# akshilpatel/tile-match-gym

Hardware: AMD Instinct MI355X
Metric: env-steps/sec (whole node), 65536×10×10 boards, at 1/2/4/8 MI355X (higher is better)
Workload: dtype int8; 1 GPU; c2: 65536 x 10x10 boards per GPU, 4 colours, no specials, num_moves=30, autoreset, 3 episode-phase blocks offset by 10 steps, the timed window opening on a block's reset step (phases + 4); boards_per_gpu=65536, rows=10, cols=10, colours=4, env_groups_per_gpu=3, phase_blocks=3, policy=uniform, api=raw, graph=False, parallelism=dp1 (independent env shards, no collective)

## Files before the change

tile-match-gym_amd/csrc/tmg_board.hip:

```cpp
#include <hip/hip_runtime.h>
#include <stdint.h>

#include "pcg64.h"

namespace tmg {

#define WSYNC() __syncthreads()

#ifndef TMG_LEAN128_WAVES
#define TMG_LEAN128_WAVES 8
#endif
constexpr int kLean128Waves = TMG_LEAN128_WAVES;
constexpr int kLean128GenericWaves = 7;
constexpr int kGen128Waves = 5;
#ifndef TMG_RESET512_WAVES
#define TMG_RESET512_WAVES 8
#endif
#ifndef TMG_RESET128_WAVES
#define TMG_RESET128_WAVES 8
#endif
constexpr int kReset512Waves = TMG_RESET512_WAVES;
constexpr int kReset128Waves = TMG_RESET128_WAVES;
#ifndef TMG_PEEK_LEAN_WAVES
#define TMG_PEEK_LEAN_WAVES 5
// ... 53 lines not shown
    CV_SPILL,
    CV_SPILL_RUN,
    CV_SHUFFLE,
    CV_REJECT,
    CV_FAST,
    CV_SHUFFLE_GEN,
    CV_REJECT_GEN,
    CV_RP_PASSES,
    CV_RP_PERP,
    CV_RP_VLONG,
    CV_RP_WIDE,
    CV_RP_REJECT,
    CV_LANE_STEP,
    CV_LANE_SHUFFLE,
    CV_LANE_REDRAW,
    CV_LANE_REJECT,
    CV_LANE_REJECT_REDRAW,
    CV_RP_CARRY,
    CV_RP_REBATCH,
    CV_PEEK_MOVE,
    CV_PEEK_SPILL,
    CV_PEEK_SPILL_RUN,
    CV_ROLL_PLY,
    CV_ROLL_HORIZON,
    CV_ROLL_SPILL,
    CV_ROLL_SPILL_RUN,
    CV_BP_PAIR_ACC,
    CV_BP_PAIR_REJ,
    CV_RP_VSHIFT,
    CV_RP_VMORE,
    CV_RP_SCAN2,
    CV_BP_ROUND_CARRY,
    CV_RP_NOLDS,
    CV_COUNT = 48
};
#if TMG_COVER
#define COVER(site)                                                                                     \
    do {                                                                                                \
        if (lane == 0 && P.cover) atomicAdd(P.cover + (site), 1ULL);                                   \
    } while (0)
#define COVER_L0(site)                                                                                  \
    do {                                                                                                \
        if (P.cover) atomicAdd(P.cover + (site), 1ULL);                                                \
    } while (0)
#else
#define COVER(site) ((void)0)
#define COVER_L0(site) ((void)0)
#endif

struct Params {
    int R, C, N, A, W, k, smask, num_moves;
    uint32_t thr;
    uint32_t cmag, cm1mag;
    const uint64_t *jump;
    uint64_t sb_nl[2];
    uint64_t sb_nf[2];
    uint64_t sb_h[2];
    uint64_t sb_z;
    uint64_t sb_in[2], sb_u[2], sb_v[2];
    const uint64_t *sb_rows;
    uint32_t *status;
    void *oh;
    int oh_dtype, oh_ch, oh_nsel;
    uint32_t oh_sel;
    SpillQ *spill;
    void *spill_ws;
    unsigned long long *cover;
// ... 2148 lines not shown
    return elim;
}

struct JumpRow { uint64_t a0, a1, g0, g1; };
__device__ __forceinline__ JumpRow jump_row_load(const Params &P, int l, bool rowp) {
    const uint64_t *t = P.jump + (rowp ? bp_out(l) : l) * 4;
    return JumpRow{t[0], t[1], t[2], t[3]};
}
__device__ __forceinline__ LaneJump jump_row_finish(const JumpRow &r, const Rng &g) {
    LaneJump J;
    J.Aj = U128{r.a0, r.a1};
    J.Gj = U128{r.g0, r.g1};
    J.incG = mul128(U128{g.ilo, g.ihi}, J.Gj);
    return J;
}
__device__ __forceinline__ LaneJump load_jump(const Params &P, int lane, const Rng &g, bool rowp = false) {
    return jump_row_finish(jump_row_load(P, lane, rowp), g);
}
__device__ __forceinline__ LaneJump load_jump_bp(const Params &P, int lane, const Rng &g) {
    return load_jump(P, lane, g, true);
}

__device__ __forceinline__ Rng load_rng(const uint64_t *p) {
    Rng g;
    g.slo = bcast64(p[0]); g.shi = bcast64(p[1]); g.ilo = bcast64(p[2]); g.ihi = bcast64(p[3]); g.h = bcast64(p[4]);
    return g;
}
__device__ __forceinline__ void store_rng(uint64_t *p, const Rng &g, int lane) {
    if (lane == 0) { p[0] = g.slo; p[1] = g.shi; p[2] = g.ilo; p[3] = g.ihi; p[4] = g.h; }
}

#include "tmg_rp.hip"

template <int MAXN, bool GEN, int SBNB, bool CODD, int TIER = TIER_MAIN, class WS = Ws<MAXN, GEN>,
          class L = WsSerial<MAXN>, bool FIXED = false>
__device__ __forceinline__ uint32_t step_env(
    const Params &P, WS &w, int lane, int64_t e, int8_t *__restrict__ board, uint64_t *__restrict__ rng, int32_t *__restrict__ timer,
    const int32_t *__restrict__ actions, int32_t *__restrict__ reward, int32_t *__restrict__ n_new,
    int32_t *__restrict__ n_act, uint8_t *__restrict__ flags_out, uint64_t *__restrict__ eff, int trust_eff,
    int autoreset, L *lists) {
    const int N = P.N, W = P.W;
    constexpr bool INLINE_GEN = !GEN && MAXN == 128;
    const bool same = autoreset == 1 || autoreset == 2;
    const bool regen_inline = autoreset == 1 || autoreset == 3;
    int a = __builtin_amdgcn_readfirstlane(actions[e]);
    const int t0 = __builtin_amdgcn_readfirstlane(timer[e]);
    const uint64_t effrow = lane < W ? eff[e * W + lane] : 0ULL;
    TMG_KEEP_V(effrow);
    if (P.sample) {
        a = __builtin_amdgcn_readfirstlane(sample_action(P, effrow, e, lane));
        if (lane == 0) const_cast<int32_t *>(actions)[e] = a;
    }
#ifndef TMG_QEXIT
#define TMG_QEXIT 1
#endif
    if (TMG_QEXIT && trust_eff && t0 < P.num_moves - 1 && (unsigned)a < (unsigned)P.A) {
        if (!((rdlane64(effrow, a >> 6) >> (a & 63)) & 1ULL)) {
            if (lane == 0) {
                uint64_t ve = (uint64_t)e;
                TMG_OPAQUE_V(ve);
                timer[ve] = t0 + 1;
                reward[ve] = 0; n_new[ve] = 0; n_act[ve] = 0;
                flags_out[ve] = (uint8_t)0;
                if (P.vo_term) reinterpret_cast<uint32_t *>(P.vo_term)[ve] = 0u;
                if (P.vo_left) P.vo_left[ve] = (int64_t)(P.num_moves - 1 - t0);
            }
            return 0;
        }
    }
    bool pend = false;
    if (t0 >= P.num_moves || a < 0 || a >= P.A) {
        pend = autoreset >= 3 && t0 >= P.num_moves;
    }
    if (!pend && (t0 >= P.num_moves || a < 0 || a >= P.A)) {
        if (lane == 0) {
            reward[e] = 0; n_new[e] = 0; n_act[e] = 0; flags_out[e] = FL_ERR;
            store_vo(P, e, FL_ERR, t0);
        }
        if ((P.oh || P.vo_obs) && !trust_eff) {
            load_board(P, w, lane, board + e * 2 * N);
            WSYNC();
            if (P.oh) store_onehot(P, w, lane, e);
            if (P.vo_obs) store_obs(P, w, lane, e);
        }
        return ST_CALLER;
    }
    int8_t *gb = board + e * 2 * N;
    uint64_t *ge = eff + e * W;
    const int t1 = t0 + 1;
    const bool done = !pend && t1 == P.num_moves;
    const bool regen = pend || (done && same);
    int flags = done ? FL_DONE : 0;
    bool effective = false;
    if (trust_eff && !pend) {
        effective = (rdlane64(effrow, a >> 6) >> (a & 63)) & 1ULL;
    }
    if (trust_eff && !effective && !(regen && regen_inline)) {
        const bool defer = regen;
        if (done && !same) {
            for (int i = lane; i < W; i += 64) ge[i] = 0ULL;
            if (P.vo_mask) store_mask(P, w, lane, e, true);
        }
        if (done && same && P.vo_final) {
            const int nbw = ((2 * N) & 3) == 0 ? (2 * N) >> 2 : 0;
            const uint32_t *src = reinterpret_cast<const uint32_t *>(gb);
            uint32_t *dst = reinterpret_cast<uint32_t *>(P.vo_final + e * 2 * N);
            for (int i = lane; i < nbw; i += 64) dst[i] = src[i];
            for (int i = 4 * nbw + lane; i < 2 * N; i += 64) P.vo_final[e * 2 * N + i] = gb[i];
        }
        if (lane == 0) {
            const int tn = defer ? 0 : t1;
            timer[e] = tn; reward[e] = 0; n_new[e] = 0; n_act[e] = 0;
            flags_out[e] = (uint8_t)(flags | (defer ? FL_RESET : 0));
            store_vo(P, e, flags, tn);
        }
        return 0;
    }
    int r1, c1, r2, c2;
    action_coords(P.R, P.C, a, r1, c1, r2, c2);
    const int p1 = r1 * P.C + c1, p2 = r2 * P.C + c2;

    const int nbw = (2 * N) >> 2;
    const bool bwhole = ((2 * N) & 3) == 0 && nbw <= 64;
    const uint32_t bw = bwhole ? reinterpret_cast<const uint32_t *>(gb)[lane < nbw ? lane : 0] : 0u;
    const uint64_t *rp = rng + e * 5;
    const uint64_t q0 = rp[0], q1 = rp[1], q2 = rp[2], q3 = rp[3], q4 = rp[4];
    bool rowp = false;
    if constexpr (SBNB > 0 && !GEN) rowp = rp_shape(P);
    const JumpRow jrow = jump_row_load(P, lane, rowp);
    if (bwhole) {
        if (lane < nbw) reinterpret_cast<uint32_t *>(w.brd)[lane] = bw;
    } else {
        load_board(P, w, lane, gb);
    }
    if constexpr (GEN) {
        for (int p = lane; p < N; p += 64) w.mark[p] = 0;
    }
    if constexpr (TIER == TIER_SPILL) COVER(CV_SPILL_RUN);
    WSYNC();
    if constexpr (!GEN) {
        bool ok = true;
        for (int p = lane; p < N; p += 64) ok &= w.brd[N + p] == 1;
        if (__ballot(!ok) != 0ULL) {
            if (lane == 0) {
                reward[e] = 0; n_new[e] = 0; n_act[e] = 0; flags_out[e] = FL_ERR;
                store_vo(P, e, FL_ERR, t0);
            }
            return ST_INTERNAL;
        }
    }
    if (!trust_eff && !pend) {
        bool ex = lane == 0 ? eff_exact(P, w.brd, a) : false;
        effective = __ballot(ex) != 0ULL;
    }
    Rng g;
    g.slo = bcast64(q0); g.shi = bcast64(q1); g.ilo = bcast64(q2); g.ihi = bcast64(q3); g.h = bcast64(q4);
    LaneJump J = jump_row_finish(jrow, g);
    const Cells<MAXN / 64> cl = make_cells<MAXN / 64>(P, lane);
    int elim = 0, nn = 0, na = 0;
    bool changed = false;
    if (effective) {
        if constexpr (SBNB > 0 && !GEN) {
            bool nolds = false;
            if constexpr (INLINE_GEN)
                nolds = regen && regen_inline && P.C <= 32 && !P.vo_final && !P.oh && !P.vo_obs;
            if (rowp) elim = rp_move<SBNB, CODD, kRpLevers>(P, w, lane, J, g, cl, p1, p2, flags, nolds);
            else elim = sb_move<SBNB, CODD>(P, w, lane, J, g, cl, p1, p2, flags, e);
        } else elim = board_move<MAXN, GEN, SBNB, CODD, TIER>(P, w, lane, J, g, cl, p1, p2, flags, nn, na, e, lists,
                                                             trust_eff != 0);
        changed = true;
        if constexpr (GEN) {
            if (flags & FL_OVF) {
                if constexpr (TIER == TIER_MAIN) {
                    if (queue_env(P.spill, lane, e)) { COVER(CV_SPILL); return 0; }
                }
                flags = (flags & ~FL_OVF) | FL_ERR;
            }
        }
    }
    int tnew = t1;
    if (regen) {
        if (done && P.vo_final) store_board(P, w, lane, P.vo_final + e * 2 * N);
        if constexpr (INLINE_GEN) {
            if (regen_inline) {
                int fg = -1;
                if constexpr (SBNB > 0) {
                    if (P.C <= 32) fg = bp_generate<SBNB, true, FIXED>(P, w, lane, g);
                    if (fg < 0) {
                        if (rowp) J = load_jump(P, lane, g);
                        fg = sb_generate_exact<SBNB, CODD>(P, w, lane, J, g, cl);
                    }
                } else {
                    fg = generate_board(P, w, lane, J, g, cl);
                }
                flags |= fg;
                changed = true;
            }
        }
        tnew = 0;
        flags |= FL_RESET;
    }
    if (changed) {
        store_board(P, w, lane, gb);
        store_rng(rng + e * 5, g, lane);
    }
    if (P.oh && (changed || !trust_eff)) store_onehot(P, w, lane, e);
    if (P.vo_obs && (changed || !trust_eff)) store_obs(P, w, lane, e);
    if (done && !same) {
        for (int i = lane; i < W; i += 64) ge[i] = 0ULL;
        if (P.vo_mask) store_mask(P, w, lane, e, true);
    } else if (changed) {
        for (int i = lane; i < W; i += 64) ge[i] = w.effw[i];
        if (P.vo_mask) store_mask(P, w, lane, e, false);
    } else if (!trust_eff) {
        scan_effective(P, w, lane, cl, false);
        WSYNC();
        for (int i = lane; i < W; i += 64) ge[i] = w.effw[i];
        if (P.vo_mask) store_mask(P, w, lane, e, false);
    }
    if (lane == 0) {
        timer[e] = tnew;
        reward[e] = elim;
        n_new[e] = nn;
        n_act[e] = na;
        flags_out[e] = (uint8_t)flags;
        store_vo(P, e, flags, tnew);
    }
    return ((flags & FL_ERR) ? ST_INTERNAL : 0u) | ((flags & FL_OVF) ? ST_OVERFLOW : 0u);
}

#if defined(__clang__)
#define TMG_ASSUME(x) __builtin_assume(x)
#else
#define TMG_ASSUME(x) do { if (!(x)) __builtin_unreachable(); } while (0)
#endif
constexpr int shape_fix(int R, int C, int k, int smask) { return (R << 24) | (C << 16) | (k << 8) | smask; }
constexpr int kNoFix = 0;
constexpr int kFixAnySpecials = 255;
constexpr int kFixC2 = shape_fix(10, 10, 4, 0);
constexpr int kFixC3 = shape_fix(10, 10, 4, SP_VLASER | SP_HLASER | SP_BOMB);
constexpr int kFixC5 = shape_fix(20, 20, 6, SP_COOKIE | SP_VLASER | SP_HLASER | SP_BOMB);
constexpr int kFixReset10 = shape_fix(10, 10, 4, kFixAnySpecials);
constexpr int kFixReset20 = shape_fix(20, 20, 6, kFixAnySpecials);
__host__ __device__ constexpr uint64_t fix_mask(int R, int C, int w, int what) {
    uint64_t m = 0;
    for (int p = 0; p < R * C && p < 128; p++) {
        const int c = p % C;
        if ((p & 1) != w) continue;
        const bool on = what == 0 ? true : what == 1 ? p >= C : what == 2 ? p >= 2 * C : what == 3 ? c <= C - 2
                      : what == 4 ? c >= 1 : c <= C - 3;
        if (on) m |= 1ULL << (p >> 1);
    }
    return m;
}
template <int FIX>
__device__ __forceinline__ void assume_shape(const Params &P) {
    if constexpr (FIX != kNoFix) {
        constexpr struct { int R, C, K, smask; } F{FIX >> 24, (FIX >> 16) & 255, (FIX >> 8) & 255, FIX & 255};
        TMG_ASSUME(P.R == F.R);
        TMG_ASSUME(P.C == F.C);
        TMG_ASSUME(P.N == F.R * F.C);
// ... 11 lines not shown
        TMG_ASSUME(P.field[0] == m0);                                   \
        TMG_ASSUME(P.field[1] == m1);                                   \
    }
            TMG_ASSUME_MASK(sb_in, 0)
            TMG_ASSUME_MASK(sb_u, 1)
            TMG_ASSUME_MASK(sb_v, 2)
            TMG_ASSUME_MASK(sb_nl, 3)
            TMG_ASSUME_MASK(sb_nf, 4)
            TMG_ASSUME_MASK(sb_h, 5)
#undef TMG_ASSUME_MASK
        }
    }
}

template <int MAXN, bool GEN, int SBNB = 0, bool CODD = false, int FIX = kNoFix>
__global__ __launch_bounds__(64, MAXN == 128 ? (GEN ? kGen128Waves : (FIX != kNoFix ? kLean128Waves : kLean128GenericWaves))
                                            : (FIX == kFixC5 ? kC5StepWaves : 1)) void step_kernel(
    Params P_, int64_t n, int8_t *__restrict__ board, uint64_t *__restrict__ rng, int32_t *__restrict__ timer,
    const int32_t *__restrict__ actions, int32_t *__restrict__ reward, int32_t *__restrict__ n_new,
    int32_t *__restrict__ n_act, uint8_t *__restrict__ flags_out, uint64_t *__restrict__ eff, int trust_eff,
    int autoreset) {
    TMG_SMEM_DECL(smem);
    using WS = Ws<MAXN, GEN>;
    const Params &P = TMG_KERNARG_PARAMS(P_);
    assume_shape<FIX>(P);
    const int lane = threadIdx.x & 63;
    WS &w = *reinterpret_cast<WS *>(smem);
    const int64_t e = wg_env();
    if (e >= n) return;
    WsSerial<MAXN> *lists = nullptr;
    if constexpr (GEN) lists = &w.s;
    const uint32_t st = step_env<MAXN, GEN, SBNB, CODD, TIER_MAIN, WS, WsSerial<MAXN>, FIX != kNoFix>(
        P, w, lane, e, board, rng, timer, actions, reward, n_new, n_act, flags_out, eff, trust_eff, autoreset, lists);
    note_status(P, lane, st);
}

template <int MAXN, class Body>
__device__ __forceinline__ void spill_drain(const Params &P, int64_t limit, Body body) {
    TMG_SMEM_DECL(smem);
    using WS = Ws<MAXN, false>;
    const int lane = threadIdx.x & 63;
    WS &w = *reinterpret_cast<WS *>(smem);
    SpillQ *q = P.spill;
    WsSerialBig<MAXN> *lists = reinterpret_cast<WsSerialBig<MAXN> *>(P.spill_ws) + blockIdx.x;
    const int64_t queued = (int64_t)(uint32_t)__builtin_amdgcn_readfirstlane((int)q->count);
    const int cnt = (int)(queued < q->cap ? queued : q->cap);
    int done = 0;
    for (int i = (int)blockIdx.x; i < cnt; i += (int)gridDim.x) {
        const int64_t id = (int64_t)bcast64((uint64_t)q->env[i]);
        if (id < 0 || id >= limit) continue;
        WSYNC();
        note_status(P, lane, body(w, lane, id, lists));
        done++;
    }
    if (lane == 0) {
        if (done) atomicAdd(&q->total, (unsigned long long)done);
        __threadfence();
        if (atomicAdd(&q->done, 1u) == gridDim.x - 1) { q->count = 0u; q->done = 0u; }
    }
}

template <int MAXN>
__global__ __launch_bounds__(64, 8) void spill_kernel(
    Params P, int64_t n, int8_t *__restrict__ board, uint64_t *__restrict__ rng, int32_t *__restrict__ timer,
    const int32_t *__restrict__ actions, int32_t *__restrict__ reward, int32_t *__restrict__ n_new,
    int32_t *__restrict__ n_act, uint8_t *__restrict__ flags_out, uint64_t *__restrict__ eff, int trust_eff,
// ... 84 lines not shown
```

tile-match-gym_amd/csrc/tmg_capi.hip:

```cpp
#include <hip/hip_runtime.h>

#include <cstdio>
#include <cstdlib>
#include <cstring>
#include <mutex>
#include <string>
#include <utility>
#include <vector>

#include "tmg.h"
#include "tmg_board.hip"
#include "tmg_dispatch.h"
#include "tmg_expand.hip"
#include "tmg_launch.h"
#include "tmg_seed.h"

#ifndef TMG_SRC_SHA
#define TMG_SRC_SHA "unknown"
#endif
#ifndef TMG_VARIANT
#define TMG_VARIANT "product"
#endif

namespace {
// ... 84 lines not shown
    }
    *q = sp->q;
    *ws = sp->ws;
    return 0;
}

static int set_device(tmg_ctx *ctx) {
    int dev = 0;
    (void)hipGetDevice(&dev);
    if (dev != ctx->device) return hip_check(hipSetDevice(ctx->device), "hipSetDevice");
    return 0;
}

static int do_reset(tmg_ctx *ctx, const Params &P, int64_t n, int8_t *board, uint64_t *rng, int32_t *timer,
                    uint64_t *eff, const uint8_t *env_mask, int mask_bits, hipStream_t s, int epw) {
    const dim3 grid = tmg::env_grid((n + epw - 1) / epw);
    if (ctx->maxn == 128) tmg::launch_reset128(ctx->sb, grid, s, P, n, board, rng, timer, eff, env_mask, mask_bits, epw);
    else tmg::launch_reset512(grid, s, P, n, board, rng, timer, eff, env_mask, mask_bits, epw);
    return hip_check(hipGetLastError(), "kernel launch");
}

static int do_step(tmg_ctx *ctx, Params P, StepArgs a, hipStream_t s) {
    const tmg::StepRoute r = tmg::route_step(P, ctx->maxn, a.trust_eff, a.autoreset, a.n, true);
    const dim3 grid = tmg::env_grid(a.n);
    if (r.spill) {
        int rc = spill_for(ctx, s, a.n, &P.spill, &P.spill_ws);
        if (rc) return rc;
    }
    a.autoreset = r.kernel_autoreset;
    if (r.lane) {
        tmg::launch_step_lane(s, P, a);
    } else {
        switch (tmg::step_group(P, ctx->maxn, ctx->sb, r.lean)) {
        case tmg::StepGroup::Lean128: tmg::launch_step_lean128(ctx->sb, grid, s, P, a); break;
        case tmg::StepGroup::Gen128Even: tmg::launch_step_gen128_even(ctx->sb, grid, s, P, a); break;
        case tmg::StepGroup::Gen128Odd: tmg::launch_step_gen128_odd(grid, s, P, a); break;
        case tmg::StepGroup::Step512: tmg::launch_step512(!r.lean, grid, s, P, a); break;
        }
    }
    int rc = hip_check(hipGetLastError(), "kernel launch");
    if (rc) return rc;
    if (r.spill) {
        if (ctx->maxn == 128) tmg::launch_spill128(s, P, a);
        else tmg::launch_spill512(s, P, a);
        rc = hip_check(hipGetLastError(), "kernel launch");
        if (rc) return rc;
    }
    if (!r.deferred) return 0;
    return do_reset(ctx, P, a.n, a.board, a.rng, a.timer, a.eff, a.flags, tmg::FL_RESET, s, r.reset_epw);
}

static int check_call(tmg_ctx *ctx, int64_t n) {
    if (!ctx) return fail(-1, "null context");
    if (n < 0) return fail(-2, "negative batch size");
    return set_device(ctx);
}

static int check_full(tmg_ctx *ctx, int64_t n) {
    int rc = check_call(ctx, n);
    if (!rc && ctx->scan_only) return fail(-2, "context made by tmg_create_scan: tmg_effective only");
    return rc;
}

namespace {

bool has_line(const int *b, int R, int C) {
    for (int r = 0; r < R; r++)
// ... 756 lines not shown
```

tile-match-gym_amd/csrc/tmg_dispatch.h:

```cpp
#pragma once
#include <stdint.h>

namespace tmg {


#ifndef TMG_LANE
#define TMG_LANE 1
#endif
#ifndef TMG_LANE_MIN_ENVS
#define TMG_LANE_MIN_ENVS 131072
#endif
constexpr bool kLaneKernel = TMG_LANE != 0;
constexpr int64_t kLaneMinEnvs = TMG_LANE_MIN_ENVS;
#ifndef TMG_LANE_SMALL
#define TMG_LANE_SMALL 32768
#endif
constexpr int64_t kLaneSmallEnvs = TMG_LANE_SMALL;
#ifndef TMG_LANE_RESET_EPW
#define TMG_LANE_RESET_EPW 2
#endif
constexpr int kLaneResetEnvs = TMG_LANE_RESET_EPW;
constexpr int kMaskedResetEnvs128 = 8;
constexpr int kMaskedResetEnvs512 = 2;
#ifndef TMG_GEN_SAMPLE
#define TMG_GEN_SAMPLE 0
#endif
constexpr bool kGenSampleInKernel = TMG_GEN_SAMPLE != 0;

inline int shape_maxn(const Params &P) { return P.N <= 128 ? 128 : 512; }
inline bool shape_sb(const Params &P) { return P.N <= 128 && P.C <= 63; }
inline bool lane_shape(const Params &P) {
    return P.smask == 0 && P.R == 10 && P.C == 10 && (P.k == 4 || P.k == 5);
}
inline bool fused_output(const Params &P) {
    return P.oh || P.vo_term || P.vo_mask || P.vo_left || P.vo_final || P.vo_obs;
}

inline bool lean_step(const Params &P, int trust_eff) { return P.smask == 0 && trust_eff; }

inline int reset_envs_per_wave(int maxn, bool masked, int override = 0) {
    return !masked ? 1 : override ? override : maxn == 128 ? kMaskedResetEnvs128 : kMaskedResetEnvs512;
}

inline bool sample_ahead(const Params &P, int trust_eff) {
    return P.sample && !kGenSampleInKernel && !lean_step(P, trust_eff);
}

struct StepRoute {
    bool lean;
    bool lane;
    bool deferred;
    bool spill;
    int kernel_autoreset;
    int reset_epw;
};

inline StepRoute route_step(const Params &P, int maxn, int trust_eff, int mode, int64_t n, bool have_lane) {
    StepRoute r;
    r.lean = lean_step(P, trust_eff);
    r.lane = have_lane && kLaneKernel && r.lean && maxn == 128 && lane_shape(P) && !fused_output(P) &&
             (P.sample || n >= kLaneMinEnvs);
    r.deferred = mode && (maxn == 512 || !r.lean || r.lane);
    r.spill = !r.lean;
    r.kernel_autoreset = mode == 0 ? 0 : mode == 1 ? (r.deferred ? 2 : 1) : (r.deferred ? 4 : 3);
    r.reset_epw = r.deferred ? reset_envs_per_wave(maxn, true, r.lane ? kLaneResetEnvs : 0) : 0;
    return r;
}

enum class StepGroup { Lean128, Gen128Even, Gen128Odd, Step512 };
inline StepGroup step_group(const Params &P, int maxn, bool sb, bool lean) {
    if (maxn != 128) return StepGroup::Step512;
    if (lean) return StepGroup::Lean128;
    return sb && (P.C & 1) ? StepGroup::Gen128Odd : StepGroup::Gen128Even;
}


template <int FIX>
bool is_shape(const Params &P) {
    const int sm = (FIX & 255) == kFixAnySpecials ? kFixAnySpecials : P.smask;
    return shape_fix(P.R, P.C, P.k, sm) == FIX;
}

template <bool GEN, bool CODD, class L>
void step_sb_ladder(const Params &P, L &l) {
    switch (sb_planes(P.k)) {
    case 1: l.template step<128, GEN, 1, CODD, kNoFix>(); break;
    case 2: l.template step<128, GEN, 2, CODD, kNoFix>(); break;
    case 3: l.template step<128, GEN, 3, CODD, kNoFix>(); break;
    default: l.template step<128, GEN, 4, CODD, kNoFix>(); break;
    }
}

template <class L>
void step_lean128_ladder(const Params &P, bool sb, L &l) {
    if (!sb) l.template step<128, false, 0, false, kNoFix>();
    else if (is_shape<kFixC2>(P)) l.template step<128, false, 2, false, kFixC2>();
    else if (P.C & 1) step_sb_ladder<false, true>(P, l);
    else step_sb_ladder<false, false>(P, l);
}

template <class L>
void step_gen128_even_ladder(const Params &P, bool sb, L &l) {
    if (!sb) l.template step<128, true, 0, false, kNoFix>();
    else if (is_shape<kFixC3>(P)) l.template step<128, true, 2, false, kFixC3>();
    else step_sb_ladder<true, false>(P, l);
}

template <class L>
void step_gen128_odd_ladder(const Params &P, L &l) {
    step_sb_ladder<true, true>(P, l);
}

template <class L>
void step512_ladder(const Params &P, bool gen, L &l) {
    if (!gen) l.template step<512, false, 0, false, kNoFix>();
    else if (is_shape<kFixC5>(P)) l.template step<512, true, 0, false, kFixC5>();
    else l.template step<512, true, 0, false, kNoFix>();
}

template <bool CODD, class L>
void reset_sb_ladder(const Params &P, L &l) {
    switch (sb_planes(P.k)) {
    case 1: l.template reset<128, 1, CODD, kNoFix>(); break;
    case 2: l.template reset<128, 2, CODD, kNoFix>(); break;
    case 3: l.template reset<128, 3, CODD, kNoFix>(); break;
    default: l.template reset<128, 4, CODD, kNoFix>(); break;
    }
}
// ... 14 lines not shown
    case 2: l.template reset<512, 2, false, kNoFix>(); break;
    case 3: l.template reset<512, 3, false, kNoFix>(); break;
    default: l.template reset<512, 4, false, kNoFix>(); break;
    }
}

template <bool GEN, bool CODD, class L>
void peek_sb_ladder(const Params &P, L &l) {
    switch (sb_planes(P.k)) {
    case 1: l.template peek<128, GEN, 1, CODD>(); break;
    case 2: l.template peek<128, GEN, 2, CODD>(); break;
    case 3: l.template peek<128, GEN, 3, CODD>(); break;
    default: l.template peek<128, GEN, 4, CODD>(); break;
    }
}
template <bool GEN, class L>
void peek_group_ladder(const Params &P, int maxn, bool sb, L &l) {
    if (maxn != 128) l.template peek<512, GEN, 0, false>();
    else if (!sb) l.template peek<128, GEN, 0, false>();
    else if (P.C & 1) peek_sb_ladder<GEN, true>(P, l);
    else peek_sb_ladder<GEN, false>(P, l);
}
template <class L>
void peek_lean_ladder(const Params &P, int maxn, bool sb, L &l) { peek_group_ladder<false>(P, maxn, sb, l); }
template <class L>
void peek_gen_ladder(const Params &P, int maxn, bool sb, L &l) { peek_group_ladder<true>(P, maxn, sb, l); }

template <class L>
void effective128_ladder(L &l) { l.template effective<128>(); }
template <class L>
void effective512_ladder(L &l) { l.template effective<512>(); }

template <class L>
void step_ladder(const Params &P, int maxn, bool sb, bool lean, L &l) {
    switch (step_group(P, maxn, sb, lean)) {
    case StepGroup::Lean128: step_lean128_ladder(P, sb, l); break;
    case StepGroup::Gen128Even: step_gen128_even_ladder(P, sb, l); break;
    case StepGroup::Gen128Odd: step_gen128_odd_ladder(P, l); break;
    case StepGroup::Step512: step512_ladder(P, !lean, l); break;
    }
}
template <class L>
void reset_ladder(const Params &P, int maxn, bool sb, L &l) {
    if (maxn == 128) reset128_ladder(P, sb, l);
    else reset512_ladder(P, l);
}
template <class L>
void peek_ladder(const Params &P, int maxn, bool sb, bool lean, L &l) {
    if (lean) peek_lean_ladder(P, maxn, sb, l);
    else peek_gen_ladder(P, maxn, sb, l);
}
template <class L>
void effective_ladder(int maxn, L &l) {
    if (maxn == 128) effective128_ladder(l);
    else effective512_ladder(l);
}

}
```

tile-match-gym_amd/csrc/tmg_kernels.hip:

```cpp
#include <hip/hip_runtime.h>

#include "tmg_board.hip"
#include "tmg_dispatch.h"
#include "tmg_launch.h"
#if TMG_TU == 1
#if TMG_COVER
#define TMG_LANE_COVER_PTR 1
#define TMG_LANE_COVER(g, site)                                                                         \
    do {                                                                                                \
        if ((g).cover) atomicAdd((g).cover + (tmg::CV_LANE_STEP + (site)), 1ULL);                       \
    } while (0)
#endif
#include "tmg_lane.h"
#endif
#if TMG_TU == 6
#include "tmg_aux.hip"
#endif

#if TMG_TU == 12
#include "tmg_expand.hip"
#endif

#ifndef TMG_TU
#error "compile tmg_kernels.hip with -DTMG_TU=1..15"
#endif

namespace tmg {

namespace {

struct StepLaunch {
    dim3 grid;
    hipStream_t s;
    const Params &P;
    const StepArgs &a;
    template <int MAXN, bool GEN, int NB, bool CODD, int FIX>
    void step() {
        const size_t lds = sizeof(Ws<MAXN, GEN>);
        hipLaunchKernelGGL((step_kernel<MAXN, GEN, NB, CODD, FIX>), grid, dim3(64), lds, s, P, a.n, a.board, a.rng,
                           a.timer, a.actions, a.reward, a.n_new, a.n_act, a.flags, a.eff, a.trust_eff, a.autoreset);
    }
};

template <int MAXN>
void spill_one(hipStream_t s, const Params &P, const StepArgs &a) {
    const size_t lds = sizeof(Ws<MAXN, false>);
    hipLaunchKernelGGL((spill_kernel<MAXN>), dim3(kSpillWaves), dim3(64), lds, s, P, a.n, a.board, a.rng, a.timer,
                       a.actions, a.reward, a.n_new, a.n_act, a.flags, a.eff, a.trust_eff, a.autoreset);
}

struct ResetLaunch {
    dim3 grid;
    hipStream_t s;
    const Params &P;
    int64_t n;
    int8_t *board;
    uint64_t *rng;
    int32_t *timer;
    uint64_t *eff;
    const uint8_t *env_mask;
    int mask_bits, epw;
    template <int MAXN, int NB, bool CODD, int FIX>
    void reset() {
        const size_t lds = sizeof(Ws<MAXN, false>);
        hipLaunchKernelGGL((reset_kernel<MAXN, NB, CODD, FIX>), grid, dim3(64), lds, s, P, n, board, rng, timer, eff,
                           env_mask, mask_bits, epw);
    }
};

struct EffectiveLaunch {
    dim3 grid;
    hipStream_t s;
    const Params &P;
// ... 168 lines not shown
    const Params &P = TMG_KERNARG_PARAMS(P_);
    const int lane = threadIdx.x & 63;
    const int64_t e = wg_env() * EPW + lane;
    if (lane >= EPW || e >= n) return;
    static_assert(CV_LANE_STEP + lane::LC_COUNT <= CV_COUNT &&
                      CV_LANE_REJECT_REDRAW - CV_LANE_STEP == lane::LC_REJECT_REDRAW,
                  "CV_LANE_* follow tmg_lane.h's LC_* order");
#if TMG_COVER
    const lane::StepIO io{board, rng, timer, actions, reward, n_new, n_act, flags, eff,
                          P.num_moves, autoreset, P.sample, P.pol_key, P.pol_first, P.pol_t, P.cover};
#else
    const lane::StepIO io{board, rng, timer, actions, reward, n_new, n_act, flags, eff,
                          P.num_moves, autoreset, P.sample, P.pol_key, P.pol_first, P.pol_t};
#endif
    const uint32_t st = lane::step_env<lane::Board<R, C, K>>(io, e, scratch + lane * kLaneScratch);
    if (st & lane::LS_INTERNAL) P.status[0] = 1u;
    if (st & lane::LS_CALLER) P.status[2] = 1u;
}

template <int K, int EPW>
void lane_one(hipStream_t s, const Params &P, const StepArgs &a) {
    const dim3 grid = env_grid((a.n + EPW - 1) / EPW);
    int32_t *act = const_cast<int32_t *>(a.actions);
    hipLaunchKernelGGL((lane_step_kernel<10, 10, K, EPW>), grid, dim3(64), 0, s, P, a.n, a.board, a.rng, a.timer,
                       act, a.reward, a.n_new, a.n_act, a.flags, a.eff, a.autoreset);
}

void launch_step_lane(hipStream_t s, const Params &P, const StepArgs &a) {
    const bool small = a.n < kLaneSmallEnvs;
    if (P.k == 4) small ? lane_one<4, 32>(s, P, a) : lane_one<4, 64>(s, P, a);
    else small ? lane_one<5, 32>(s, P, a) : lane_one<5, 64>(s, P, a);
}

void launch_step_lean128(bool sb, dim3 grid, hipStream_t s, const Params &P, const StepArgs &a) {
    StepLaunch l{grid, s, P, a};
    step_lean128_ladder(P, sb, l);
}
#endif

#if TMG_TU == 2
void launch_step_gen128_even(bool sb, dim3 grid, hipStream_t s, const Params &P, const StepArgs &a) {
    StepLaunch l{grid, s, P, a};
    step_gen128_even_ladder(P, sb, l);
}
#endif

#if TMG_TU == 7
void launch_spill128(hipStream_t s, const Params &P, const StepArgs &a) { spill_one<128>(s, P, a); }
void launch_spill512(hipStream_t s, const Params &P, const StepArgs &a) { spill_one<512>(s, P, a); }
#endif

#if TMG_TU == 3
void launch_step_gen128_odd(dim3 grid, hipStream_t s, const Params &P, const StepArgs &a) {
    StepLaunch l{grid, s, P, a};
    step_gen128_odd_ladder(P, l);
}
#endif

#if TMG_TU == 4
void launch_step512(bool gen, dim3 grid, hipStream_t s, const Params &P, const StepArgs &a) {
    StepLaunch l{grid, s, P, a};
    step512_ladder(P, gen, l);
}

void launch_reset512(dim3 grid, hipStream_t s, const Params &P, int64_t n, int8_t *board, uint64_t *rng,
                     int32_t *timer, uint64_t *eff, const uint8_t *env_mask, int mask_bits, int epw) {
    ResetLaunch l{grid, s, P, n, board, rng, timer, eff, env_mask, mask_bits, epw};
    reset512_ladder(P, l);
}
// ... 62 lines not shown
```

tile-match-gym_amd/csrc/tmg_launch.h:

```cpp
#pragma once
#include <hip/hip_runtime.h>
#include <stddef.h>
#include <stdint.h>

namespace tmg {

struct Params;

struct StepArgs {
    int64_t n;
    int8_t *board;
    uint64_t *rng;
    int32_t *timer;
    const int32_t *actions;
    int32_t *reward, *n_new, *n_act;
    uint8_t *flags;
    uint64_t *eff;
    int trust_eff, autoreset;
};

dim3 env_grid(int64_t n);

void launch_step_lean128(bool sb, dim3 grid, hipStream_t s, const Params &P, const StepArgs &a);
void launch_step_lane(hipStream_t s, const Params &P, const StepArgs &a);
constexpr int kLaneScratch = 128;
void launch_step_gen128_even(bool sb, dim3 grid, hipStream_t s, const Params &P, const StepArgs &a);
void launch_step_gen128_odd(dim3 grid, hipStream_t s, const Params &P, const StepArgs &a);
void launch_step512(bool gen, dim3 grid, hipStream_t s, const Params &P, const StepArgs &a);
void launch_spill128(hipStream_t s, const Params &P, const StepArgs &a);
void launch_spill512(hipStream_t s, const Params &P, const StepArgs &a);
void launch_reset512(dim3 grid, hipStream_t s, const Params &P, int64_t n, int8_t *board, uint64_t *rng,
                     int32_t *timer, uint64_t *eff, const uint8_t *env_mask, int mask_bits, int epw);
void launch_effective512(dim3 grid, hipStream_t s, const Params &P, int64_t n, const int8_t *board, uint64_t *eff);
void launch_reset128(bool sb, dim3 grid, hipStream_t s, const Params &P, int64_t n, int8_t *board, uint64_t *rng,
                     int32_t *timer, uint64_t *eff, const uint8_t *env_mask, int mask_bits, int epw);
void launch_effective128(dim3 grid, hipStream_t s, const Params &P, int64_t n, const int8_t *board, uint64_t *eff);
void launch_onehot(hipStream_t s, int64_t n, int N, int k, int nsel, int4 sel, const int8_t *board, void *out,
                   int dtype);
void launch_sample_effective(hipStream_t s, int64_t n, int W, int A, const uint64_t *eff, uint64_t key,
                             int64_t first_env, int32_t t, int32_t *actions);
void launch_count_states(int R, int C, int k, uint64_t total, uint64_t per, uint64_t threads,
                         unsigned long long *counts);
struct SeedArgs;
void launch_seed(hipStream_t s, const SeedArgs &a, int store);

struct PeekArgs {
    int64_t n;
    const int8_t *board;
    const uint64_t *rng;
    const uint64_t *eff;
    int trust_eff;
    int32_t *reward, *n_new, *n_act;
    uint8_t *flags;
    int32_t *best_action, *best_reward;
};
void launch_peek_lean(int maxn, bool sb, dim3 grid, hipStream_t s, const Params &P, const PeekArgs &a);
// ... 33 lines not shown
```

tile-match-gym_amd/tile_match_gym_amd/_native.py:

```python
from __future__ import annotations

import ctypes
import hashlib
import os

from . import _buildinfo

_HERE = os.path.dirname(os.path.abspath(__file__))
DEFAULT_LIB = os.path.join(_HERE, "_lib", "libtmg.so")
LIB_PATH = os.environ.get("TMG_LIB") or DEFAULT_LIB
EXPORTS = ("tmg_create", "tmg_create_scan", "tmg_destroy", "tmg_reset", "tmg_step", "tmg_effective",
           "tmg_num_actions", "tmg_mask_words", "tmg_last_error", "tmg_abi_version", "tmg_build_info",
           "tmg_onehot", "tmg_onehot_channels", "tmg_count_states", "tmg_sample_effective", "tmg_status",
           "tmg_viable", "tmg_spills", "tmg_step_onehot", "tmg_reset_onehot", "tmg_plan_create", "tmg_plan_config",
           "tmg_plan_step", "tmg_plan_join", "tmg_plan_destroy", "tmg_plan_capture", "tmg_graph_launch",
           "tmg_graph_destroy", "tmg_peek", "tmg_rollout", "tmg_seed", "tmg_expand_count", "tmg_expand",
           "tmg_playout", "tmg_trace")
DTYPE_F32, DTYPE_U8, DTYPE_I32 = 0, 1, 2
ABI_VERSION = 10
SEED_INT, SEED_SPAWN, SEED_STORE_DIRECT, SEED_STORE_STAGED = 0, 1, 0x100, 0x200
STATUS_INTERNAL, STATUS_OVERFLOW, STATUS_CALLER = 1, 2, 4

COVER_NAMES = ("sb_lean", "sb_normal", "sb_laser", "sb_perp_bomb", "sb_row_bomb", "sb_closure", "sb_fallback",
               "lds_normal", "lds_laser", "lds_bomb", "lds_fallback", "serial_step", "serial_act", "serial_cookie",
               "combo", "spill", "spill_run", "shuffle", "reject", "fast", "shuffle_gen", "reject_gen",
               "rp_passes", "rp_perp", "rp_vlong", "rp_wide", "rp_reject",
               "lane_step", "lane_shuffle", "lane_redraw", "lane_reject", "lane_reject_redraw",
               "rp_carry", "rp_rebatch", "peek_move", "peek_spill", "peek_spill_run",
               "roll_ply", "roll_horizon", "roll_spill", "roll_spill_run",
               "bp_pair_acc", "bp_pair_rej", "rp_vshift", "rp_vmore", "rp_scan2", "bp_round_carry", "rp_nolds")

SPECIAL_BITS = {"cookie": 1, "vertical_laser": 2, "horizontal_laser": 4, "bomb": 8}
FLAG_DONE, FLAG_COMBO, FLAG_SHUFFLED, FLAG_RESET, FLAG_OVERFLOW, FLAG_ERROR = 1, 2, 4, 8, 0x40, 0x80
FLAG_STOPPED = 0x10
STAGE_SWAP, STAGE_COMBO, STAGE_CLEAR, STAGE_FALL, STAGE_REFILL, STAGE_SHUFFLE = 1, 2, 3, 4, 5, 6
STAGE_NAMES = {STAGE_SWAP: "swap", STAGE_COMBO: "combo", STAGE_CLEAR: "clear", STAGE_FALL: "fall",
               STAGE_REFILL: "refill", STAGE_SHUFFLE: "shuffle"}

_libs = {}
_M64 = (1 << 64) - 1

P = ctypes.c_void_p
I = ctypes.c_int
I64 = ctypes.c_int64
U64 = ctypes.c_uint64


class TmgError(RuntimeError):
    pass


def load(path: str = None):
    path = path or LIB_PATH
    L = _libs.get(path)
    if L is not None:
        return L
    if not os.path.exists(path):
        raise TmgError(f"{path} not found: build it with `make -C tile-match-gym_amd` "
                       "(or __graft_entry__.build()); there is no CPU fallback")
    L = ctypes.CDLL(path)
    L.tmg_create.argtypes = [ctypes.POINTER(P), I, I, I, I, ctypes.c_uint32, I]
    L.tmg_create_scan.argtypes = [ctypes.POINTER(P), I, I, I]
    L.tmg_build_info.argtypes = []
# ... 308 lines not shown
```

Baseline: 1.346 billion env-steps/s.

## Add specialized plain step kernel for lean 10x10 no-special shape

Adds a dedicated plain_step_kernel for the c2 shape (lean, no specials, no fused outputs, no sampling). It takes its hot pointers in a compact kernarg struct, reads Params straight from the kernarg segment, and uses 32-bit byte offsets. It checks the action against the effective mask in scalar registers and ends the wave early for ineffective actions. Inside step_env it compiles out the fused-output branches. The aim is to cut per-wave scalar setup, 64-bit address arithmetic and branch overhead on the common quick-exit path, at the cost of another kernel variant and a limit on the number of envs.

```diff
diff --git a/tile-match-gym_amd/csrc/tmg_board.hip b/tile-match-gym_amd/csrc/tmg_board.hip
--- a/tile-match-gym_amd/csrc/tmg_board.hip
+++ b/tile-match-gym_amd/csrc/tmg_board.hip
@@ -109,7 +109,9 @@
     CV_RP_SCAN2,
     CV_BP_ROUND_CARRY,
     CV_RP_NOLDS,
-    CV_COUNT = 48
+    CV_PLAIN_EXIT,
+    CV_PLAIN_STEP,
+    CV_COUNT = 50
 };
 #if TMG_COVER
 #define COVER(site)                                                                                     \
@@ -2324,20 +2326,54 @@
 
 #include "tmg_rp.hip"
 
+struct PlainPre {
+    int a, t0, num_moves;
+    bool effective;
+};
+template <class T>
+__device__ __forceinline__ T *env_row32(T *base, int64_t e, int per) {
+    const uint32_t off = (uint32_t)e * (uint32_t)(per * (int)sizeof(T));
+    return (T *)((const char *)base + off);
+}
+__device__ __forceinline__ void plain_store_outputs(int64_t e, int32_t *__restrict__ timer,
+                                                    int32_t *__restrict__ reward, int32_t *__restrict__ n_new,
+                                                    int32_t *__restrict__ n_act, uint8_t *__restrict__ flags_out,
+                                                    int tnew, int elim, int nn, int na, int flags) {
+    uint32_t v4 = 4u * (uint32_t)e, v1 = (uint32_t)e;
+    TMG_OPAQUE_V(v4);
+    TMG_OPAQUE_V(v1);
+    *(int32_t *)((char *)timer + v4) = tnew;
+    *(int32_t *)((char *)reward + v4) = elim;
+    *(int32_t *)((char *)n_new + v4) = nn;
+    *(int32_t *)((char *)n_act + v4) = na;
+    *((uint8_t *)flags_out + v1) = (uint8_t)flags;
+}
+
 template <int MAXN, bool GEN, int SBNB, bool CODD, int TIER = TIER_MAIN, class WS = Ws<MAXN, GEN>,
-          class L = WsSerial<MAXN>, bool FIXED = false>
+          class L = WsSerial<MAXN>, bool FIXED = false, bool PLAIN = false>
 __device__ __forceinline__ uint32_t step_env(
     const Params &P, WS &w, int lane, int64_t e, int8_t *__restrict__ board, uint64_t *__restrict__ rng, int32_t *__restrict__ timer,
     const int32_t *__restrict__ actions, int32_t *__restrict__ reward, int32_t *__restrict__ n_new,
-    int32_t *__restrict__ n_act, uint8_t *__restrict__ flags_out, uint64_t *__restrict__ eff, int trust_eff,
-    int autoreset, L *lists) {
+    int32_t *__restrict__ n_act, uint8_t *__restrict__ flags_out, uint64_t *__restrict__ eff, int trust_eff_,
+    int autoreset, L *lists, const PlainPre *pre = nullptr) {
+    static_assert(!PLAIN || (!GEN && MAXN == 128 && SBNB > 0 && TIER == TIER_MAIN), "PLAIN: a lean bitboard step kernel");
     const int N = P.N, W = P.W;
+    const int trust_eff = PLAIN ? 1 : trust_eff_;
+#define TMG_FUSED(f) (!PLAIN && P.f)
+#define TMG_NUM_MOVES (PLAIN ? pre->num_moves : P.num_moves)
     constexpr bool INLINE_GEN = !GEN && MAXN == 128;
     const bool same = autoreset == 1 || autoreset == 2;
     const bool regen_inline = autoreset == 1 || autoreset == 3;
-    int a = __builtin_amdgcn_readfirstlane(actions[e]);
-    const int t0 = __builtin_amdgcn_readfirstlane(timer[e]);
-    const uint64_t effrow = lane < W ? eff[e * W + lane] : 0ULL;
+    int a, t0;
+    if constexpr (PLAIN) {
+        a = pre->a; t0 = pre->t0;
+    } else {
+        a = __builtin_amdgcn_readfirstlane(actions[e]);
+        t0 = __builtin_amdgcn_readfirstlane(timer[e]);
+    }
+    uint64_t effrow = 0ULL;
+    if constexpr (!PLAIN) {
+    effrow = lane < W ? eff[e * W + lane] : 0ULL;
     TMG_KEEP_V(effrow);
     if (P.sample) {
         a = __builtin_amdgcn_readfirstlane(sample_action(P, effrow, e, lane));
@@ -2346,7 +2382,7 @@
 #ifndef TMG_QEXIT
 #define TMG_QEXIT 1
 #endif
-    if (TMG_QEXIT && trust_eff && t0 < P.num_moves - 1 && (unsigned)a < (unsigned)P.A) {
+    if (TMG_QEXIT && trust_eff && t0 < TMG_NUM_MOVES - 1 && (unsigned)a < (unsigned)P.A) {
         if (!((rdlane64(effrow, a >> 6) >> (a & 63)) & 1ULL)) {
             if (lane == 0) {
                 uint64_t ve = (uint64_t)e;
@@ -2355,45 +2391,52 @@
                 reward[ve] = 0; n_new[ve] = 0; n_act[ve] = 0;
                 flags_out[ve] = (uint8_t)0;
                 if (P.vo_term) reinterpret_cast<uint32_t *>(P.vo_term)[ve] = 0u;
-                if (P.vo_left) P.vo_left[ve] = (int64_t)(P.num_moves - 1 - t0);
+                if (P.vo_left) P.vo_left[ve] = (int64_t)(TMG_NUM_MOVES - 1 - t0);
             }
             return 0;
         }
     }
+    }
     bool pend = false;
-    if (t0 >= P.num_moves || a < 0 || a >= P.A) {
-        pend = autoreset >= 3 && t0 >= P.num_moves;
-    }
-    if (!pend && (t0 >= P.num_moves || a < 0 || a >= P.A)) {
+    if (t0 >= TMG_NUM_MOVES || a < 0 || a >= P.A) {
+        pend = autoreset >= 3 && t0 >= TMG_NUM_MOVES;
+    }
+    if (!pend && (t0 >= TMG_NUM_MOVES || a < 0 || a >= P.A)) {
         if (lane == 0) {
             reward[e] = 0; n_new[e] = 0; n_act[e] = 0; flags_out[e] = FL_ERR;
-            store_vo(P, e, FL_ERR, t0);
-        }
-        if ((P.oh || P.vo_obs) && !trust_eff) {
+            if constexpr (!PLAIN) store_vo(P, e, FL_ERR, t0);
+        }
+        if ((TMG_FUSED(oh) || TMG_FUSED(vo_obs)) && !trust_eff) {
             load_board(P, w, lane, board + e * 2 * N);
             WSYNC();
-            if (P.oh) store_onehot(P, w, lane, e);
-            if (P.vo_obs) store_obs(P, w, lane, e);
+            if (TMG_FUSED(oh)) store_onehot(P, w, lane, e);
+            if (TMG_FUSED(vo_obs)) store_obs(P, w, lane, e);
         }
         return ST_CALLER;
     }
-    int8_t *gb = board + e * 2 * N;
-    uint64_t *ge = eff + e * W;
+    int8_t *gb;
+    uint64_t *ge, *grng;
+    if constexpr (PLAIN) {
+        gb = env_row32(board, e, 2 * N); ge = env_row32(eff, e, W); grng = env_row32(rng, e, 5);
+    } else {
+        gb = board + e * 2 * N; ge = eff + e * W; grng = nullptr;
+    }
     const int t1 = t0 + 1;
-    const bool done = !pend && t1 == P.num_moves;
+    const bool done = !pend && t1 == TMG_NUM_MOVES;
     const bool regen = pend || (done && same);
     int flags = done ? FL_DONE : 0;
     bool effective = false;
     if (trust_eff && !pend) {
-        effective = (rdlane64(effrow, a >> 6) >> (a & 63)) & 1ULL;
+        if constexpr (PLAIN) effective = pre->effective;
+        else effective = (rdlane64(effrow, a >> 6) >> (a & 63)) & 1ULL;
     }
     if (trust_eff && !effective && !(regen && regen_inline)) {
         const bool defer = regen;
         if (done && !same) {
             for (int i = lane; i < W; i += 64) ge[i] = 0ULL;
-            if (P.vo_mask) store_mask(P, w, lane, e, true);
-        }
-        if (done && same && P.vo_final) {
+            if (TMG_FUSED(vo_mask)) store_mask(P, w, lane, e, true);
+        }
+        if (done && same && TMG_FUSED(vo_final)) {
             const int nbw = ((2 * N) & 3) == 0 ? (2 * N) >> 2 : 0;
             const uint32_t *src = reinterpret_cast<const uint32_t *>(gb);
             uint32_t *dst = reinterpret_cast<uint32_t *>(P.vo_final + e * 2 * N);
@@ -2402,9 +2445,13 @@
         }
         if (lane == 0) {
             const int tn = defer ? 0 : t1;
-            timer[e] = tn; reward[e] = 0; n_new[e] = 0; n_act[e] = 0;
-            flags_out[e] = (uint8_t)(flags | (defer ? FL_RESET : 0));
-            store_vo(P, e, flags, tn);
+            if constexpr (PLAIN) {
+                plain_store_outputs(e, timer, reward, n_new, n_act, flags_out, tn, 0, 0, 0, flags | (defer ? FL_RESET : 0));
+            } else {
+                timer[e] = tn; reward[e] = 0; n_new[e] = 0; n_act[e] = 0;
+                flags_out[e] = (uint8_t)(flags | (defer ? FL_RESET : 0));
+                store_vo(P, e, flags, tn);
+            }
         }
         return 0;
     }
@@ -2415,7 +2462,9 @@
     const int nbw = (2 * N) >> 2;
     const bool bwhole = ((2 * N) & 3) == 0 && nbw <= 64;
     const uint32_t bw = bwhole ? reinterpret_cast<const uint32_t *>(gb)[lane < nbw ? lane : 0] : 0u;
-    const uint64_t *rp = rng + e * 5;
+    const uint64_t *rp;
+    if constexpr (PLAIN) rp = grng;
+    else rp = rng + e * 5;
     const uint64_t q0 = rp[0], q1 = rp[1], q2 = rp[2], q3 = rp[3], q4 = rp[4];
     bool rowp = false;
     if constexpr (SBNB > 0 && !GEN) rowp = rp_shape(P);
@@ -2436,7 +2485,7 @@
         if (__ballot(!ok) != 0ULL) {
             if (lane == 0) {
                 reward[e] = 0; n_new[e] = 0; n_act[e] = 0; flags_out[e] = FL_ERR;
-                store_vo(P, e, FL_ERR, t0);
+                if constexpr (!PLAIN) store_vo(P, e, FL_ERR, t0);
             }
             return ST_INTERNAL;
         }
@@ -2455,7 +2504,7 @@
         if constexpr (SBNB > 0 && !GEN) {
             bool nolds = false;
             if constexpr (INLINE_GEN)
-                nolds = regen && regen_inline && P.C <= 32 && !P.vo_final && !P.oh && !P.vo_obs;
+                nolds = regen && regen_inline && P.C <= 32 && !TMG_FUSED(vo_final) && !TMG_FUSED(oh) && !TMG_FUSED(vo_obs);
             if (rowp) elim = rp_move<SBNB, CODD, kRpLevers>(P, w, lane, J, g, cl, p1, p2, flags, nolds);
             else elim = sb_move<SBNB, CODD>(P, w, lane, J, g, cl, p1, p2, flags, e);
         } else elim = board_move<MAXN, GEN, SBNB, CODD, TIER>(P, w, lane, J, g, cl, p1, p2, flags, nn, na, e, lists,
@@ -2472,7 +2521,7 @@
     }
     int tnew = t1;
     if (regen) {
-        if (done && P.vo_final) store_board(P, w, lane, P.vo_final + e * 2 * N);
+        if (done && TMG_FUSED(vo_final)) store_board(P, w, lane, P.vo_final + e * 2 * N);
         if constexpr (INLINE_GEN) {
             if (regen_inline) {
                 int fg = -1;
@@ -2494,31 +2543,38 @@
     }
     if (changed) {
         store_board(P, w, lane, gb);
-        store_rng(rng + e * 5, g, lane);
-    }
-    if (P.oh && (changed || !trust_eff)) store_onehot(P, w, lane, e);
-    if (P.vo_obs && (changed || !trust_eff)) store_obs(P, w, lane, e);
+        if constexpr (PLAIN) store_rng(grng, g, lane);
+        else store_rng(rng + e * 5, g, lane);
+    }
+    if (TMG_FUSED(oh) && (changed || !trust_eff)) store_onehot(P, w, lane, e);
+    if (TMG_FUSED(vo_obs) && (changed || !trust_eff)) store_obs(P, w, lane, e);
     if (done && !same) {
         for (int i = lane; i < W; i += 64) ge[i] = 0ULL;
-        if (P.vo_mask) store_mask(P, w, lane, e, true);
+        if (TMG_FUSED(vo_mask)) store_mask(P, w, lane, e, true);
     } else if (changed) {
         for (int i = lane; i < W; i += 64) ge[i] = w.effw[i];
-        if (P.vo_mask) store_mask(P, w, lane, e, false);
+        if (TMG_FUSED(vo_mask)) store_mask(P, w, lane, e, false);
     } else if (!trust_eff) {
         scan_effective(P, w, lane, cl, false);
         WSYNC();
         for (int i = lane; i < W; i += 64) ge[i] = w.effw[i];
-        if (P.vo_mask) store_mask(P, w, lane, e, false);
+        if (TMG_FUSED(vo_mask)) store_mask(P, w, lane, e, false);
     }
     if (lane == 0) {
-        timer[e] = tnew;
-        reward[e] = elim;
-        n_new[e] = nn;
-        n_act[e] = na;
-        flags_out[e] = (uint8_t)flags;
-        store_vo(P, e, flags, tnew);
+        if constexpr (PLAIN) {
+            plain_store_outputs(e, timer, reward, n_new, n_act, flags_out, tnew, elim, nn, na, flags);
+        } else {
+            timer[e] = tnew;
+            reward[e] = elim;
+            n_new[e] = nn;
+            n_act[e] = na;
+            flags_out[e] = (uint8_t)flags;
+            store_vo(P, e, flags, tnew);
+        }
     }
     return ((flags & FL_ERR) ? ST_INTERNAL : 0u) | ((flags & FL_OVF) ? ST_OVERFLOW : 0u);
+#undef TMG_FUSED
+#undef TMG_NUM_MOVES
 }
 
 #if defined(__clang__)
@@ -2596,6 +2652,71 @@
     if constexpr (GEN) lists = &w.s;
     const uint32_t st = step_env<MAXN, GEN, SBNB, CODD, TIER_MAIN, WS, WsSerial<MAXN>, FIX != kNoFix>(
         P, w, lane, e, board, rng, timer, actions, reward, n_new, n_act, flags_out, eff, trust_eff, autoreset, lists);
+    note_status(P, lane, st);
+}
+
+struct PlainHot {
+    int32_t n;
+    int32_t per;
+    int32_t last_move;
+    int32_t autoreset;
+    const int32_t *actions;
+    int32_t *timer;
+    uint64_t *eff;
+    int32_t *reward, *n_new, *n_act;
+    uint8_t *flags;
+    int8_t *board;
+    uint64_t *rng;
+};
+static_assert(sizeof(PlainHot) % alignof(Params) == 0, "Params follows PlainHot in the kernarg segment unpadded");
+#if defined(__HIP_DEVICE_COMPILE__)
+#define TMG_PIN_S3(x, y, z) asm("" : "+s"(x), "+s"(y), "+s"(z))
+#define TMG_END_WAVE() __builtin_amdgcn_endpgm()
+#else
+#define TMG_PIN_S3(x, y, z) ((void)0)
+#define TMG_END_WAVE() return
+#endif
+#ifndef TMG_KERNARG_PARAMS_AT
+#if defined(__HIP_DEVICE_COMPILE__)
+#define TMG_KERNARG_PARAMS_AT(p, off) \
+    (*(const Params *)((const char *)__builtin_amdgcn_kernarg_segment_ptr() + (off)))
+#else
+#define TMG_KERNARG_PARAMS_AT(p, off) (p)
+#endif
+#endif
+
+template <int FIX>
+__global__ __launch_bounds__(64, kLean128Waves) void plain_step_kernel(PlainHot H, Params P_) {
+    constexpr int R = FIX >> 24, C = (FIX >> 16) & 255, K = (FIX >> 8) & 255;
+    constexpr int A = 2 * R * C - R - C, W = (A + 63) / 64;
+    static_assert(FIX != kNoFix && (FIX & 255) == 0 && R * C <= 128 && C <= 28 && !(C & 1) && W <= 3,
+                  "a lean row-plane shape with an even C and at most three mask words");
+    TMG_SMEM_DECL(smem);
+    using WS = Ws<128, false>;
+    const Params &P = TMG_KERNARG_PARAMS_AT(P_, sizeof(PlainHot));
+    assume_shape<FIX>(P);
+    const int lane = threadIdx.x & 63;
+    const uint32_t b = blockIdx.x;
+    const uint32_t e = (b & 7u) * (uint32_t)H.per + (b >> 3);
+    if (e >= (uint32_t)H.n) return;
+    const int a = __builtin_amdgcn_readfirstlane(*env_row32(H.actions, e, 1));
+    const int t0 = __builtin_amdgcn_readfirstlane(*env_row32(H.timer, e, 1));
+    const uint64_t *row = env_row32(H.eff, e, W);
+    uint64_t w0 = bcast64(row[0]), w1 = W > 1 ? bcast64(row[1]) : 0ULL, w2 = W > 2 ? bcast64(row[2]) : 0ULL;
+    TMG_PIN_S3(w0, w1, w2);
+    const uint64_t word = a < 64 ? w0 : a < 128 ? w1 : w2;
+    const uint32_t bit = (uint32_t)(word >> (a & 63)) & 1u;
+    if (t0 < H.last_move && (unsigned)a < (unsigned)A && !bit) {
+        COVER(CV_PLAIN_EXIT);
+        if (lane == 0) plain_store_outputs(e, H.timer, H.reward, H.n_new, H.n_act, H.flags, t0 + 1, 0, 0, 0, 0);
+        TMG_END_WAVE();
+    }
+    COVER(CV_PLAIN_STEP);
+    WS &w = *reinterpret_cast<WS *>(smem);
+    const PlainPre pre{a, t0, H.last_move + 1, bit != 0u};
+    const uint32_t st = step_env<128, false, sb_planes(K), false, TIER_MAIN, WS, WsSerial<128>, true, true>(
+        P, w, lane, (int64_t)e, H.board, H.rng, H.timer, H.actions, H.reward, H.n_new, H.n_act, H.flags, H.eff, 1,
+        H.autoreset, (WsSerial<128> *)nullptr, &pre);
     note_status(P, lane, st);
 }
 
diff --git a/tile-match-gym_amd/csrc/tmg_capi.hip b/tile-match-gym_amd/csrc/tmg_capi.hip
--- a/tile-match-gym_amd/csrc/tmg_capi.hip
+++ b/tile-match-gym_amd/csrc/tmg_capi.hip
@@ -140,7 +140,7 @@
         tmg::launch_step_lane(s, P, a);
     } else {
         switch (tmg::step_group(P, ctx->maxn, ctx->sb, r.lean)) {
-        case tmg::StepGroup::Lean128: tmg::launch_step_lean128(ctx->sb, grid, s, P, a); break;
+        case tmg::StepGroup::Lean128: tmg::launch_step_lean128(ctx->sb, r.plain, grid, s, P, a); break;
         case tmg::StepGroup::Gen128Even: tmg::launch_step_gen128_even(ctx->sb, grid, s, P, a); break;
         case tmg::StepGroup::Gen128Odd: tmg::launch_step_gen128_odd(grid, s, P, a); break;
         case tmg::StepGroup::Step512: tmg::launch_step512(!r.lean, grid, s, P, a); break;
diff --git a/tile-match-gym_amd/csrc/tmg_dispatch.h b/tile-match-gym_amd/csrc/tmg_dispatch.h
--- a/tile-match-gym_amd/csrc/tmg_dispatch.h
+++ b/tile-match-gym_amd/csrc/tmg_dispatch.h
@@ -38,6 +38,24 @@
 
 inline bool lean_step(const Params &P, int trust_eff) { return P.smask == 0 && trust_eff; }
 
+template <int FIX>
+bool is_shape(const Params &P) {
+    const int sm = (FIX & 255) == kFixAnySpecials ? kFixAnySpecials : P.smask;
+    return shape_fix(P.R, P.C, P.k, sm) == FIX;
+}
+
+constexpr int64_t kPlainMaxEnvs = 1 << 23;
+constexpr int64_t plain_max_offset(int R, int C) {
+    const int64_t N = R * C, W = (2 * N - R - C + 63) / 64;
+    const int64_t row = 2 * N > 40 ? (2 * N > 8 * W ? 2 * N : 8 * W) : (40 > 8 * W ? 40 : 8 * W);
+    return kPlainMaxEnvs * row;
+}
+static_assert(plain_max_offset(kFixC2 >> 24, (kFixC2 >> 16) & 255) < (1LL << 31),
+              "every env's byte offset (e * 2N, e * 40, e * 8W, e * 4) stays below 2^31");
+inline bool plain_step(const Params &P, int trust_eff, int64_t n) {
+    return is_shape<kFixC2>(P) && lean_step(P, trust_eff) && !P.sample && !fused_output(P) && n <= kPlainMaxEnvs;
+}
+
 inline int reset_envs_per_wave(int maxn, bool masked, int override = 0) {
     return !masked ? 1 : override ? override : maxn == 128 ? kMaskedResetEnvs128 : kMaskedResetEnvs512;
 }
@@ -49,6 +67,7 @@
 struct StepRoute {
     bool lean;
     bool lane;
+    bool plain;
     bool deferred;
     bool spill;
     int kernel_autoreset;
@@ -60,6 +79,7 @@
     r.lean = lean_step(P, trust_eff);
     r.lane = have_lane && kLaneKernel && r.lean && maxn == 128 && lane_shape(P) && !fused_output(P) &&
              (P.sample || n >= kLaneMinEnvs);
+    r.plain = !r.lane && maxn == 128 && plain_step(P, trust_eff, n);
     r.deferred = mode && (maxn == 512 || !r.lean || r.lane);
     r.spill = !r.lean;
     r.kernel_autoreset = mode == 0 ? 0 : mode == 1 ? (r.deferred ? 2 : 1) : (r.deferred ? 4 : 3);
@@ -75,12 +95,6 @@
 }
 
 
-template <int FIX>
-bool is_shape(const Params &P) {
-    const int sm = (FIX & 255) == kFixAnySpecials ? kFixAnySpecials : P.smask;
-    return shape_fix(P.R, P.C, P.k, sm) == FIX;
-}
-
 template <bool GEN, bool CODD, class L>
 void step_sb_ladder(const Params &P, L &l) {
     switch (sb_planes(P.k)) {
@@ -92,8 +106,9 @@
 }
 
 template <class L>
-void step_lean128_ladder(const Params &P, bool sb, L &l) {
+void step_lean128_ladder(const Params &P, bool sb, L &l, bool plain = false) {
     if (!sb) l.template step<128, false, 0, false, kNoFix>();
+    else if (is_shape<kFixC2>(P) && plain) l.template step_plain<kFixC2>();
     else if (is_shape<kFixC2>(P)) l.template step<128, false, 2, false, kFixC2>();
     else if (P.C & 1) step_sb_ladder<false, true>(P, l);
     else step_sb_ladder<false, false>(P, l);
@@ -174,9 +189,9 @@
 void effective512_ladder(L &l) { l.template effective<512>(); }
 
 template <class L>
-void step_ladder(const Params &P, int maxn, bool sb, bool lean, L &l) {
+void step_ladder(const Params &P, int maxn, bool sb, bool lean, L &l, bool plain = false) {
     switch (step_group(P, maxn, sb, lean)) {
-    case StepGroup::Lean128: step_lean128_ladder(P, sb, l); break;
+    case StepGroup::Lean128: step_lean128_ladder(P, sb, l, plain); break;
     case StepGroup::Gen128Even: step_gen128_even_ladder(P, sb, l); break;
     case StepGroup::Gen128Odd: step_gen128_odd_ladder(P, l); break;
     case StepGroup::Step512: step512_ladder(P, !lean, l); break;
diff --git a/tile-match-gym_amd/csrc/tmg_kernels.hip b/tile-match-gym_amd/csrc/tmg_kernels.hip
--- a/tile-match-gym_amd/csrc/tmg_kernels.hip
+++ b/tile-match-gym_amd/csrc/tmg_kernels.hip
@@ -39,6 +39,13 @@
         const size_t lds = sizeof(Ws<MAXN, GEN>);
         hipLaunchKernelGGL((step_kernel<MAXN, GEN, NB, CODD, FIX>), grid, dim3(64), lds, s, P, a.n, a.board, a.rng,
                            a.timer, a.actions, a.reward, a.n_new, a.n_act, a.flags, a.eff, a.trust_eff, a.autoreset);
+    }
+    template <int FIX>
+    void step_plain() {
+        const size_t lds = sizeof(Ws<128, false>);
+        const PlainHot H{(int32_t)a.n, (int32_t)(grid.x >> 3), P.num_moves - 1, a.autoreset, a.actions, a.timer, a.eff,
+                         a.reward, a.n_new, a.n_act, a.flags, a.board, a.rng};
+        hipLaunchKernelGGL((plain_step_kernel<FIX>), grid, dim3(64), lds, s, H, P);
     }
 };
 
@@ -273,9 +280,9 @@
     else small ? lane_one<5, 32>(s, P, a) : lane_one<5, 64>(s, P, a);
 }
 
-void launch_step_lean128(bool sb, dim3 grid, hipStream_t s, const Params &P, const StepArgs &a) {
+void launch_step_lean128(bool sb, bool plain, dim3 grid, hipStream_t s, const Params &P, const StepArgs &a) {
     StepLaunch l{grid, s, P, a};
-    step_lean128_ladder(P, sb, l);
+    step_lean128_ladder(P, sb, l, plain);
 }
 #endif
 
diff --git a/tile-match-gym_amd/csrc/tmg_launch.h b/tile-match-gym_amd/csrc/tmg_launch.h
--- a/tile-match-gym_amd/csrc/tmg_launch.h
+++ b/tile-match-gym_amd/csrc/tmg_launch.h
@@ -21,7 +21,7 @@
 
 dim3 env_grid(int64_t n);
 
-void launch_step_lean128(bool sb, dim3 grid, hipStream_t s, const Params &P, const StepArgs &a);
+void launch_step_lean128(bool sb, bool plain, dim3 grid, hipStream_t s, const Params &P, const StepArgs &a);
 void launch_step_lane(hipStream_t s, const Params &P, const StepArgs &a);
 constexpr int kLaneScratch = 128;
 void launch_step_gen128_even(bool sb, dim3 grid, hipStream_t s, const Params &P, const StepArgs &a);
diff --git a/tile-match-gym_amd/tile_match_gym_amd/_native.py b/tile-match-gym_amd/tile_match_gym_amd/_native.py
--- a/tile-match-gym_amd/tile_match_gym_amd/_native.py
+++ b/tile-match-gym_amd/tile_match_gym_amd/_native.py
@@ -28,7 +28,8 @@
                "lane_step", "lane_shuffle", "lane_redraw", "lane_reject", "lane_reject_redraw",
                "rp_carry", "rp_rebatch", "peek_move", "peek_spill", "peek_spill_run",
                "roll_ply", "roll_horizon", "roll_spill", "roll_spill_run",
-               "bp_pair_acc", "bp_pair_rej", "rp_vshift", "rp_vmore", "rp_scan2", "bp_round_carry", "rp_nolds")
+               "bp_pair_acc", "bp_pair_rej", "rp_vshift", "rp_vmore", "rp_scan2", "bp_round_carry", "rp_nolds",
+               "plain_exit", "plain_step")
 
 SPECIAL_BITS = {"cookie": 1, "vertical_laser": 2, "horizontal_laser": 4, "bomb": 8}
 FLAG_DONE, FLAG_COMBO, FLAG_SHUFFLED, FLAG_RESET, FLAG_OVERFLOW, FLAG_ERROR = 1, 2, 4, 8, 0x40, 0x80
```

Result: faster. 1.393 billion env-steps/s (median of 6 runs) (+3.5%).
